# chsl/PLADE

Hardware: AMD Instinct MI355X
Metric: scan-pair registrations/sec, 1M-pt synthetic pairs (higher is better)
Workload: dtype f32

## Files before the change

plade_amd/csrc/ctx.h:

```cpp
#pragma once
#include "common.h"
#include "plade_hip.h"
#include "launch.h"
#include <ctime>
#include <sys/prctl.h>

namespace plade {

struct CloudDev {
    uint32_t n = 0;
    DBuf<float> soa;
    DBuf<float> aos;
    size_t pitch = 0;
    float bbmin[3] = {0, 0, 0}, bbmax[3] = {0, 0, 0};
    const float *x() const { return soa.p; }
    const float *y() const { return soa.p + pitch; }
    const float *z() const { return soa.p + 2 * pitch; }
    const float *nx() const { return soa.p + 3 * pitch; }
    const float *ny() const { return soa.p + 4 * pitch; }
    const float *nz() const { return soa.p + 5 * pitch; }
};

struct Stats {
    std::vector<std::string> names;
    std::vector<double> values;
    std::string joined;
    void clear() { names.clear(); values.clear(); }
    void add(const std::string &n, double v) {
        for (size_t i = 0; i < names.size(); ++i)
            if (names[i] == n) { values[i] += v; return; }
        names.push_back(n);
        values.push_back(v);
    }
    void merge(const Stats &o) { for (size_t i = 0; i < o.names.size(); ++i) add(o.names[i], o.values[i]); }
};

}

namespace plade {
inline void poll_sleep(int polls, bool crowd = false) {
    const long base_ns = crowd ? 100000L : 50000L;
    timespec ts{0, polls < 8 ? base_ns : 2 * base_ns};
    nanosleep(&ts, nullptr);
}
inline double thread_cpu_seconds() {
    timespec ts;
    clock_gettime(CLOCK_THREAD_CPUTIME_ID, &ts);
    return (double)ts.tv_sec + 1e-9 * (double)ts.tv_nsec;
}
inline void relax_timer_slack() {
    static thread_local bool done = false;
    if (!done) { (void)prctl(PR_SET_TIMERSLACK, 1000UL, 0, 0, 0); done = true; }
}
}

namespace plade {
struct ScanWork { DBuf<uint64_t> state; DBuf<uint32_t> ticket; uint32_t base = 0, gen = 0; };
struct VoxBatchWork { DBuf<uint32_t> keys, keys2, vals, vals2, heads, seg_group, offs; DBuf<float> sorted_xyz, obb_coef; };
}

namespace plade {
constexpr int COPY_OUT_RANGES = 8;
struct CopyOutArgs { const uint32_t *src[COPY_OUT_RANGES]; uint32_t off_words[COPY_OUT_RANGES], words[COPY_OUT_RANGES], n; };
void copy_out_launch(hipStream_t st, const CopyOutArgs &a, uint32_t *arena_words, uint32_t *counter, uint32_t *flag, uint32_t seq);
}

struct plade_cloud {
    plade::CloudDev dev;
    std::vector<float> host_copy;
};

namespace plade { struct RegistrationWork; struct RansacWork; struct NormalsWork; struct IcpWork; struct DistWork; struct OutlierWork; struct MergeWork; struct ComponentWork; }
namespace plade { void comm_all_gather_dev(plade_comm *c, const void *d_send, void *d_recv, size_t bytes, hipStream_t stream); }

struct plade_ctx {
    int device = 0;
    plade::RegistrationWork *reg_work = nullptr;
    plade::RansacWork *ransac_work = nullptr;
    plade::NormalsWork *normals_work = nullptr;
    plade::IcpWork *icp_work = nullptr;
    plade::DistWork *dist_work = nullptr;
    plade::OutlierWork *outlier_work = nullptr;
    plade::MergeWork *merge_work = nullptr;
    plade::ComponentWork *component_work = nullptr;
    plade_ctx *peers[PLADE_GROUP_MAX - 1] = {};
    hipEvent_t ev_group = nullptr;
    bool in_group = false;
    const char *stage_name = "";
    plade::Combiner *comb = nullptr;
    int comb_slot = -1;
    plade_ctx *aux = nullptr;
    hipStream_t stream = nullptr;
    plade::CloudDev up_tgt, up_src;
    struct Prefetch {
        hipStream_t stream = nullptr;
        plade::CloudDev cl[2 * PLADE_GROUP_MAX];
        const float *ptr[2 * PLADE_GROUP_MAX] = {};
        uint32_t n[2 * PLADE_GROUP_MAX] = {};
        int count = 0;
        bool valid = false;
        plade::HBuf<int> h;
        plade::DBuf<int> d;
    } pf;
    plade_params params;
    struct CandidateShard { uint32_t rank = 0, world = 1, min_candidates = 0; plade_exchange_fn exchange = nullptr; void *user = nullptr;
                            plade_comm *comm = nullptr;  } shard;
    uint64_t wait_epoch = 0;
    std::string last_error;
    std::map<std::string, std::vector<char>> dump;
    plade::Stats stats;
    struct EvRec { hipEvent_t a = nullptr, b = nullptr; std::string tag; double bytes = 0; int clk = -1; double clk_secs = -1.0; };
    std::vector<EvRec> evs;
    static constexpr int CLK_SLOTS = 1024, CLK_WAYS = 64;
    plade::DBuf<unsigned long long> clk_dev;
    int clk_used = 0;
    double clk_hz = 0;
    bool graph_clocks() const { return (params.dump & 6) == 6; }
    bool capturing = false;
    int cap_slot = 0;
    std::vector<std::string> cap_tags;
    std::vector<unsigned long long> clk_host, clk_init;
    void ensure_clk() {
        if (clk_dev.p) return;
        {
            clk_dev.ensure(2 * (size_t)CLK_SLOTS * CLK_WAYS);
            std::vector<unsigned long long> init(2 * (size_t)CLK_SLOTS * CLK_WAYS);
            for (size_t i = 0; i < init.size() / 2; ++i) { init[2 * i] = ~0ull; init[2 * i + 1] = 0ull; }
            (void)hipMemcpy(clk_dev.p, init.data(), init.size() * 8, hipMemcpyHostToDevice);
            int khz = 0;
            (void)hipDeviceGetAttribute(&khz, hipDeviceAttributeWallClockRate, device);
            clk_hz = khz > 0 ? khz * 1e3 : 1e8;
        }
    }
    unsigned long long *ev_clock() {
        if (graph_clocks()) {
            if (!capturing || cap_slot >= CLK_SLOTS) return nullptr;
            ensure_clk();
            return clk_dev.p + 2 * (size_t)CLK_WAYS * (cap_slot++);
        }
        if (!profiling() || evs.empty() || clk_used >= CLK_SLOTS) return nullptr;
        ensure_clk();
        evs.back().clk = clk_used;
        return clk_dev.p + 2 * (size_t)CLK_WAYS * (clk_used++);
    }
    void ev_graph_launched(const std::vector<std::string> &tags) {
        for (size_t j = 0; j < tags.size(); ++j) { EvRec r; r.tag = tags[j]; r.clk = (int)j; evs.push_back(r); }
    }
    void ev_graph_clocks(size_t ev0) {
        size_t used = 0;
        for (size_t e = ev0; e < evs.size(); ++e) if (!evs[e].a && evs[e].clk >= 0) used = std::max(used, (size_t)evs[e].clk + 1);
        if (!used) return;
        clk_host.resize(2 * used * CLK_WAYS);
        if (clk_init.size() < clk_host.size()) {
            clk_init.resize(clk_host.size());
            for (size_t i = 0; i < clk_init.size() / 2; ++i) { clk_init[2 * i] = ~0ull; clk_init[2 * i + 1] = 0ull; }
        }
        HIP_TRY(hipMemcpyAsync(clk_host.data(), clk_dev.p, clk_host.size() * 8, hipMemcpyDeviceToHost, stream));
        HIP_TRY(hipMemcpyAsync(clk_dev.p, clk_init.data(), clk_host.size() * 8, hipMemcpyHostToDevice, stream));
        HIP_TRY(hipStreamSynchronize(stream));
        for (size_t e = ev0; e < evs.size(); ++e) {
            EvRec &r = evs[e];
            if (r.a || r.clk < 0) continue;
            unsigned long long lo = ~0ull, hi = 0ull;
            for (int w = 0; w < CLK_WAYS; ++w) {
                lo = std::min(lo, clk_host[2 * ((size_t)r.clk * CLK_WAYS + w)]);
                hi = std::max(hi, clk_host[2 * ((size_t)r.clk * CLK_WAYS + w) + 1]);
            }
            r.clk_secs = hi > lo ? (double)(hi - lo) / clk_hz : -1.0;
            r.clk = -1;
        }
    }
    bool profiling() const { return (params.dump & 2) != 0; }
    void ev_begin(const char *tag, double bytes) {
        if (!profiling()) return;
        if (graph_clocks()) { if (capturing) cap_tags.push_back(tag); return; }
        EvRec r;
        r.tag = tag; r.bytes = bytes;
        (void)hipEventCreate(&r.a); (void)hipEventCreate(&r.b);
        (void)hipEventRecord(r.a, stream);
        evs.push_back(r);
    }
    void ev_end() {
        if (!profiling() || graph_clocks() || evs.empty()) return;
        (void)hipEventRecord(evs.back().b, stream);
    }
    void ev_collect() {
        if (evs.empty()) return;
        (void)hipStreamSynchronize(stream);
        std::vector<unsigned long long> clk(2 * (size_t)clk_used);
        if (clk_used) {
            std::vector<unsigned long long> raw(2 * (size_t)clk_used * CLK_WAYS);
            (void)hipMemcpy(raw.data(), clk_dev.p, raw.size() * 8, hipMemcpyDeviceToHost);
            for (int i = 0; i < clk_used; ++i) {
                unsigned long long lo = ~0ull, hi = 0ull;
                for (int w = 0; w < CLK_WAYS; ++w) {
                    lo = std::min(lo, raw[2 * ((size_t)i * CLK_WAYS + w)]);
                    hi = std::max(hi, raw[2 * ((size_t)i * CLK_WAYS + w) + 1]);
                }
                clk[2 * i] = lo; clk[2 * i + 1] = hi;
            }
            for (size_t i = 0; i < raw.size() / 2; ++i) { raw[2 * i] = ~0ull; raw[2 * i + 1] = 0ull; }
            (void)hipMemcpy(clk_dev.p, raw.data(), raw.size() * 8, hipMemcpyHostToDevice);
            clk_used = 0;
        }
        for (auto &r : evs) {
            float ms = 0.f;
            if (!r.a) {
                if (r.bytes >= 0 && r.clk_secs >= 0) {
                    stats.add("k_" + r.tag + "_seconds", r.clk_secs);
                    stats.add("k_" + r.tag + "_launches", 1.0);
                    stats.add("k_" + r.tag + "_bytes", r.bytes);
                    stats.add("k_" + r.tag + "_clock_seconds", r.clk_secs);
                    stats.add("k_" + r.tag + "_clock_launches", 1.0);
                    stats.add("k_" + r.tag + "_clock_bytes", r.bytes);
                } else stats.add("k_" + r.tag + "_idle_launches", 1.0);
                continue;
            }
            (void)hipEventElapsedTime(&ms, r.a, r.b);
            if (r.bytes >= 0) {
                stats.add("k_" + r.tag + "_seconds", ms * 1e-3);
                stats.add("k_" + r.tag + "_launches", 1.0);
                stats.add("k_" + r.tag + "_bytes", r.bytes);
                if (r.clk >= 0 && clk[2 * r.clk + 1] > clk[2 * r.clk]) {
                    stats.add("k_" + r.tag + "_clock_seconds", (double)(clk[2 * r.clk + 1] - clk[2 * r.clk]) / clk_hz);
                    stats.add("k_" + r.tag + "_clock_launches", 1.0);
                    stats.add("k_" + r.tag + "_clock_bytes", r.bytes);
                }
            } else stats.add("k_" + r.tag + "_idle_launches", 1.0);
            (void)hipEventDestroy(r.a); (void)hipEventDestroy(r.b);
        }
        evs.clear();
    }
    void sync(hipStream_t s = nullptr) {
        if (!s) s = stream;
        if (comb && s == stream) { comb->wait(this); return; }
        if (s == stream && !pending_reads.empty()) { sync_with_reads(); return; }
        if (params.host_wait == 0) { HIP_TRY(hipStreamSynchronize(s)); }
        else {
            plade::relax_timer_slack();
            const double c0 = plade::thread_cpu_seconds();
            struct Acc { plade::Stats &st; double c0; ~Acc() { st.add("cpu_sync_polls", plade::thread_cpu_seconds() - c0); } } acc{stats, c0};
            for (int polls = 0;; ++polls) {
                const hipError_t e = hipStreamQuery(s);
                if (e == hipSuccess) break;
                if (e != hipErrorNotReady) throw plade::Err{-2, std::string("hipStreamQuery: ") + hipGetErrorString(e)};
                plade::poll_sleep(polls, in_group);
            }
        }
        if (s == stream) { finish_reads(); write_arena_used = 0; ++wait_epoch; }
    }
    struct PendingRead { void *dst; const void *src; size_t off, bytes; std::vector<char> eager; };
    bool debug_reads = getenv("PLADE_DEBUG_READS") != nullptr;
    std::vector<PendingRead> pending_reads;
    plade::HBuf<char> read_arena;
    char *read_arena_dev = nullptr;
    plade::DBuf<uint32_t> read_counter;
    uint32_t read_seq = 0;
// ... 225 lines not shown
```

plade_amd/csrc/k_penetration.hip:

```cpp
#include "stages.h"
#include "prims.h"
#include "k_svd.h"
#include <algorithm>

namespace plade {

struct PenItem {
    uint32_t k, i1, j1;
    float plane1[4];
    float sx, sy, sz, dx, dy, dz, length;
};

struct PenTables {
    const float *cand;
    const float *s_coef;
    const float *s_center;
    const float *s_four;
    const float *t_coef;
    const float *t_center;
    const float *t_four;
    uint32_t K, ps, pt;
};

template <class Meet>
__device__ __forceinline__ void edge_hit(f3 lineVec, f3 linePoint, f3 a, f3 b, f3 *out, int &n, Meet meet) {
    const f3 tl = normalized_e(b - a);
    f3 ip;
    if (!meet(lineVec, linePoint, tl, a, ip)) return;
    if (dot_e(a - ip, b - ip) > 0) return;
    if (n < 4) out[n] = ip;
    ++n;
}
template <bool ROLLED, class Meet>
__device__ __forceinline__ int edge_hits(f3 lineVec, f3 linePoint, const f3 *c, f3 *out, Meet meet) {
    int n = 0;
    if (ROLLED) {
#pragma unroll 1
        for (int i = 1; i <= 4; ++i) edge_hit(lineVec, linePoint, c[(i - 1) % 4], c[i % 4], out, n, meet);
    } else {
        for (int i = 1; i <= 4; ++i) edge_hit(lineVec, linePoint, c[(i - 1) % 4], c[i % 4], out, n, meet);
    }
    return n;
}

struct PenTriple {
    uint32_t k, i1, j1;
    float plane1[4];
    f3 lineVec, linePoint;
    f3 c[8];
};

__device__ __forceinline__ bool pen_triple(const PenTables &tb, size_t idx, float len_th, float ang_th, PenTriple &t) {
    const uint32_t j1 = (uint32_t)(idx % tb.pt), i1 = (uint32_t)((idx / tb.pt) % tb.ps), k = (uint32_t)(idx / ((size_t)tb.pt * tb.ps));
    t.k = k; t.i1 = i1; t.j1 = j1;
    const float *c = tb.cand + 12 * (size_t)k;
    m3 R;
    for (int r = 0; r < 3; ++r) for (int q = 0; q < 3; ++q) R.m[r][q] = c[3 * r + q];
    const f3 T(c[9], c[10], c[11]);
    const float T12[12] = {c[0], c[1], c[2], c[9], c[3], c[4], c[5], c[10], c[6], c[7], c[8], c[11]};
    const float *sc = tb.s_coef + 4 * (size_t)i1;
    const f3 pn = mul_e(R, f3(sc[0], sc[1], sc[2]));
    t.plane1[0] = pn.x; t.plane1[1] = pn.y; t.plane1[2] = pn.z;
    t.plane1[3] = -(-sc[3] + dot_s(pn, T));
    const f3 c2m = mul_e(R, f3(tb.s_center[3 * i1], tb.s_center[3 * i1 + 1], tb.s_center[3 * i1 + 2])) + T;
    const float *tc = tb.t_coef + 4 * (size_t)j1;
    const f3 plane_A(tc[0], tc[1], tc[2]);
    const f3 tcen(tb.t_center[3 * j1], tb.t_center[3 * j1 + 1], tb.t_center[3 * j1 + 2]);
    const double c2p = (double)((fabsf(dot_e(plane_A, c2m) + tc[3]) + fabsf(dot_e(pn, tcen) + t.plane1[3])) / 2);
    if (c2p < (double)len_th && dot_e(pn, plane_A) > ang_th) return false;
    if (!plane_plane_line(t.plane1, tc, t.lineVec, t.linePoint)) return false;
    for (int q = 0; q < 4; ++q) {
        const float *f = tb.s_four + 12 * (size_t)i1 + 3 * q;
        t.c[q] = pcl_xform(T12, f3(f[0], f[1], f[2]));
        const float *g = tb.t_four + 12 * (size_t)j1 + 3 * q;
        t.c[4 + q] = f3(g[0], g[1], g[2]);
    }
    return true;
}

__device__ __forceinline__ void pen_emit(const PenTables &tb, const PenTriple &t, const f3 *ip1, const f3 *ip2, PenItem *__restrict__ items,
                                         uint32_t *__restrict__ pair_count) {
    const f3 direc = normalized_e(ip1[1] - ip1[0]);
    const f3 inter[4] = {ip1[0], ip1[1], ip2[0], ip2[1]};
    float len[4];
    int ord[4] = {0, 1, 2, 3};
    for (int q = 0; q < 4; ++q) len[q] = dot_e(inter[q] - inter[0], direc);
    for (int a = 1; a < 4; ++a) {
        int oi = ord[a];
        float lv = len[oi];
        int b = a - 1;
        while (b >= 0 && lv < len[ord[b]]) { ord[b + 1] = ord[b]; --b; }
        ord[b + 1] = oi;
    }
    if (0 == (ord[0] / 2 - ord[1] / 2)) return;
    const f3 sp = inter[ord[1]], ep = inter[ord[2]];
    const float length = norm_e(ep - sp);
    const uint32_t pair = t.i1 * tb.pt + t.j1;
    const uint32_t slot = pair * tb.K + atomicAdd(&pair_count[pair], 1u);
    PenItem it;
    it.k = t.k; it.i1 = t.i1; it.j1 = t.j1;
    for (int q = 0; q < 4; ++q) it.plane1[q] = t.plane1[q];
    it.sx = sp.x; it.sy = sp.y; it.sz = sp.z; it.dx = direc.x; it.dy = direc.y; it.dz = direc.z; it.length = length;
    items[slot] = it;
}

template <int TPB>
__device__ void k_pen_setup(const VB &vb, PenTables tb, float len_th, float ang_th, PenItem *__restrict__ items,
                            uint32_t *__restrict__ n_items, uint32_t *__restrict__ pair_count) {
    (void)n_items;
    const size_t idx = (size_t)vb.bx * blockDim.x + threadIdx.x;
    const size_t total = (size_t)tb.K * tb.ps * tb.pt;
    if (idx >= total) return;
    PenTriple t;
    if (!pen_triple(tb, idx, len_th, ang_th, t)) return;
    f3 ip1[4], ip2[4];
    auto meet = [&](f3 v1, f3 p1, f3 v2, f3 p2, f3 &out) -> bool { return lines_meet(v1, p1, v2, p2, out); };
    const int n1 = edge_hits<false>(t.lineVec, t.linePoint, t.c, ip1, meet);
    const int n2 = edge_hits<false>(t.lineVec, t.linePoint, t.c + 4, ip2, meet);
    if (n1 != 2 || n2 != 2) return;
    pen_emit(tb, t, ip1, ip2, items, pair_count);
}

constexpr int PS_TPB = 64;
__device__ void k_pen_setup_svd(const VB &vb, PenTables tb, float len_th, float ang_th, PenItem *__restrict__ items,
                                uint32_t *__restrict__ n_items, uint32_t *__restrict__ pair_count) {
    (void)n_items;
    __shared__ float pub[54 * PS_TPB];
    __shared__ uint16_t queue[8 * PS_TPB];
    const uint32_t lane = threadIdx.x;
    const size_t idx = (size_t)vb.bx * PS_TPB + lane;
    const size_t total = (size_t)tb.K * tb.ps * tb.pt;
    PenTriple t;
    const bool active = idx < total && pen_triple(tb, idx, len_th, ang_th, t);
    uint32_t need = 0;
    auto put = [&](int w, f3 v) { pub[(w + 0) * PS_TPB + lane] = v.x; pub[(w + 1) * PS_TPB + lane] = v.y; pub[(w + 2) * PS_TPB + lane] = v.z; };
    auto get = [&](int w, uint32_t l) { return f3(pub[(w + 0) * PS_TPB + l], pub[(w + 1) * PS_TPB + l], pub[(w + 2) * PS_TPB + l]); };
    if (active) {
        put(0, t.lineVec); put(3, t.linePoint);
#pragma unroll
        for (int e = 0; e < 8; ++e) {
            const int base = e & 4, i = (e & 3) + 1;
            const f3 a = t.c[base + (i - 1) % 4], b = t.c[base + i % 4];
            const f3 tl = normalized_e(b - a);
            if (!(fabsf(dot_e(t.lineVec, tl)) > 0.9999)) {
                need |= 1u << e;
                put(6 + 6 * e, tl); put(9 + 6 * e, a);
            }
        }
    }
    uint32_t n_items_wave = 0;
#pragma unroll
    for (int e = 0; e < 8; ++e) {
        const unsigned long long m = __ballot((need >> e) & 1u);
        if ((need >> e) & 1u) queue[n_items_wave + __popcll(m & ((1ull << lane) - 1ull))] = (uint16_t)(lane | (e << 6));
        n_items_wave += (uint32_t)__popcll(m);
    }
    __syncthreads();
    for (uint32_t first = 0; first < n_items_wave; first += PS_TPB) {
        const uint32_t it = first + lane;
        if (it < n_items_wave) {
            const uint32_t q = queue[it], sl = q & 63u, e = q >> 6;
            const f3 o = lines_meet_svd(get(0, sl), get(3, sl), get(6 + 6 * e, sl), get(9 + 6 * e, sl));
            pub[(6 + 6 * e) * PS_TPB + sl] = o.x; pub[(7 + 6 * e) * PS_TPB + sl] = o.y; pub[(8 + 6 * e) * PS_TPB + sl] = o.z;
        }
    }
    __syncthreads();
    if (!active) return;
    f3 ip1[4], ip2[4];
    int n1 = 0, n2 = 0;
#pragma unroll
    for (int e = 0; e < 8; ++e) {
        if (!((need >> e) & 1u)) continue;
        const int base = e & 4, i = (e & 3) + 1;
        const f3 a = t.c[base + (i - 1) % 4], b = t.c[base + i % 4];
        const f3 ip = get(6 + 6 * e, lane);
        if (dot_e(a - ip, b - ip) > 0) continue;
        if (e < 4) { if (n1 < 4) ip1[n1] = ip; ++n1; }
        else { if (n2 < 4) ip2[n2] = ip; ++n2; }
    }
    if (n1 != 2 || n2 != 2) return;
    pen_emit(tb, t, ip1, ip2, items, pair_count);
}

constexpr int PEN_MAXS = 1024;
constexpr int PEN_G = 4;
constexpr int PEN_TPB = 64 * PEN_G;

__device__ __forceinline__ void pen_uv(const PenFrame &f, f3 p, float &u, float &v) {
    const float dx = p.x - f.o[0], dy = p.y - f.o[1], dz = p.z - f.o[2];
    u = dx * f.eu[0] + dy * f.eu[1] + dz * f.eu[2];
    v = dx * f.ev[0] + dy * f.ev[1] + dz * f.ev[2];
}

__device__ void k_pen_cell_keys(const VB &vb, const float *__restrict__ xyz, uint32_t n, const uint32_t *__restrict__ off, uint32_t P,
                                const PenFrame *__restrict__ frames, float inv_cell, uint32_t *__restrict__ keys,
                                uint32_t *__restrict__ vals) {
    const uint32_t i = vb.bx * blockDim.x + threadIdx.x;
    if (i >= n) return;
    uint32_t lo = 0, hi = P;
    while (hi - lo > 1) { const uint32_t mid = (lo + hi) >> 1; if (off[mid] <= i) lo = mid; else hi = mid; }
    const PenFrame f = frames[lo];
    float u, v;
    pen_uv(f, f3(xyz[3 * (size_t)i], xyz[3 * (size_t)i + 1], xyz[3 * (size_t)i + 2]), u, v);
    const int cu = min(max((int)floorf(u * inv_cell) + 1, 0), f.nu - 1);
    const int cv = min(max((int)floorf(v * inv_cell) + 1, 0), f.nv - 1);
    keys[i] = f.base + (uint32_t)cv * (uint32_t)f.nu + (uint32_t)cu;
    vals[i] = i;
}

__device__ void k_pen_cell_fill(const VB &vb, const float *__restrict__ xyz, const uint32_t *__restrict__ skeys,
                                const uint32_t *__restrict__ svals, uint32_t n, uint32_t n_cells,
                                float4 *__restrict__ pts, uint32_t *__restrict__ cell_start) {
    const uint32_t i = vb.bx * blockDim.x + threadIdx.x;
    if (i < n) {
        const uint32_t p = svals[i];
        pts[i] = make_float4(xyz[3 * (size_t)p], xyz[3 * (size_t)p + 1], xyz[3 * (size_t)p + 2], 0.f);
    }
    if (i <= n_cells) {
        uint32_t lo = 0, hi = n;
        while (lo < hi) { const uint32_t mid = (lo + hi) >> 1; if (skeys[mid] < i) lo = mid + 1; else hi = mid; }
        cell_start[i] = lo;
    }
}

void build_pen_grid(plade_ctx *ctx, PlaneCloudsDev &pc, const PlaneGeomHost &geom, float cell) {
    const uint32_t P = geom.P, n = pc.off[P];
    std::vector<PenFrame> fr(P);
    uint32_t total = 0;
    for (uint32_t g = 0; g < P; ++g) {
        const float *c = geom.four.data() + 12 * (size_t)g;
        PenFrame &f = fr[g];
        double eu[3], ev[3], lu = 0, lv = 0;
        for (int k = 0; k < 3; ++k) { eu[k] = (double)c[3 + k] - c[k]; ev[k] = (double)c[9 + k] - c[k]; lu += eu[k] * eu[k]; lv += ev[k] * ev[k]; }
        lu = std::sqrt(lu); lv = std::sqrt(lv);
        for (int k = 0; k < 3; ++k) {
            f.o[k] = c[k];
            f.eu[k] = lu > 0 ? (float)(eu[k] / lu) : (k == 0);
            f.ev[k] = lv > 0 ? (float)(ev[k] / lv) : (k == 1);
        }
        f.nu = (int)std::min(4096.0, std::floor(lu / cell) + 3);
        f.nv = (int)std::min(4096.0, std::floor(lv / cell) + 3);
        f.base = total;
        total += (uint32_t)f.nu * (uint32_t)f.nv;
    }
    pc.n_cells = total;
    pc.grid_cell = cell;
    pc.frames.ensure(P);
    const bool staged = ctx->h2d(pc.frames.p, fr.data(), P * sizeof(PenFrame));
    pc.cell_pts.ensure((size_t)n + 1);
    pc.cell_start.ensure((size_t)total + 2);
    pc.ckeys.ensure((size_t)n + 1); pc.ckeys2.ensure((size_t)n + 1); pc.cvals.ensure((size_t)n + 1); pc.cvals2.ensure((size_t)n + 1);
    if (n)
        launch<k_pen_cell_keys, 256>(ctx, dim3(cdiv(n, 256)), 0, pc.xyz.p, n, pc.d_off.p, P, pc.frames.p,
                           1.f / cell, pc.ckeys.p, pc.cvals.p);
    int bits = 1;
    while ((1ull << bits) < total) ++bits;
    sort_pairs_u32(ctx, pc.ckeys.p, pc.ckeys2.p, pc.cvals.p, pc.cvals2.p, n, bits);
    launch<k_pen_cell_fill, 256>(ctx, dim3(cdiv(std::max(n, total + 1), 256)), 0, pc.xyz.p, pc.ckeys2.p,
                       pc.cvals2.p, n, total, pc.cell_pts.p, pc.cell_start.p);
    if (!staged) ctx->sync();
}

template <class Fn>
__device__ __forceinline__ void pen_visit(const PenFrame &f, const float4 *__restrict__ pts, const uint32_t *__restrict__ cell_start,
                                          f3 start, f3 direc, float L, float rr, float cell, int lane, Fn fn) {
    float su, sv, eu_, ev_;
    pen_uv(f, start, su, sv);
    pen_uv(f, f3(start.x + L * direc.x, start.y + L * direc.y, start.z + L * direc.z), eu_, ev_);
    const float inv = 1.f / cell;
    const bool major_u = fabsf(eu_ - su) >= fabsf(ev_ - sv);
    const float a0 = major_u ? su : sv, a1 = major_u ? eu_ : ev_, b0 = major_u ? sv : su, b1 = major_u ? ev_ : eu_;
    const int na = major_u ? f.nu : f.nv, nbm = major_u ? f.nv : f.nu;
    const float pad = rr * 1.4143f + 0.02f * cell;
    const float amin = fminf(a0, a1) - rr - 0.02f * cell, amax = fmaxf(a0, a1) + rr + 0.02f * cell;
    const int ca0 = max((int)floorf(amin * inv) + 1, 0), ca1 = min((int)floorf(amax * inv) + 1, na - 1);
    const float da = a1 - a0;
    const float slope = fabsf(da) > 1e-12f ? (b1 - b0) / da : 0.f;
    for (int base = ca0; base <= ca1; base += 64) {
        const int ca = base + lane;
        int cb0 = 0, ncell = 0;
        if (ca <= ca1) {
            float lo = fmaxf((float)(ca - 1) * cell, amin), hi = fminf((float)ca * cell, amax);
            if (hi < lo) { const float t = lo; lo = hi; hi = t; }
            const float bl = b0 + (lo - a0) * slope, bh = b0 + (hi - a0) * slope;
            cb0 = max((int)floorf((fminf(bl, bh) - pad) * inv) + 1, 0);
            const int cb1 = min((int)floorf((fmaxf(bl, bh) + pad) * inv) + 1, nbm - 1);
            ncell = max(cb1 - cb0 + 1, 0);
        }
        int most = ncell;
        for (int d = 32; d >= 1; d >>= 1) most = max(most, __shfl_xor(most, d, 64));
        constexpr int QN = 4;
        for (int q0 = 0; q0 < most; q0 += QN) {
            uint32_t pb[QN], len[QN], mine = 0;
#pragma unroll
            for (int q = 0; q < QN; ++q) {
                pb[q] = 0; len[q] = 0;
                if (q0 + q < ncell) {
                    const int cb = cb0 + q0 + q;
                    const uint32_t c = f.base + (major_u ? (uint32_t)cb * (uint32_t)f.nu + (uint32_t)ca
                                                         : (uint32_t)ca * (uint32_t)f.nu + (uint32_t)cb);
                    pb[q] = cell_start[c];
                    len[q] = cell_start[c + 1] - pb[q];
                }
                mine += len[q];
            }
            uint32_t incl = mine;
            for (int d = 1; d < 64; d <<= 1) { const uint32_t o = __shfl_up(incl, d, 64); if (lane >= d) incl += o; }
            const uint32_t total = __shfl(incl, 63, 64), excl = incl - mine;
            for (uint32_t t0 = 0; t0 < total; t0 += 64) {
                const uint32_t t = t0 + (uint32_t)lane;
                int lo = 0, hi = 63;
                for (int it = 0; it < 6; ++it) {
                    const int mid = (lo + hi) >> 1;
                    const bool right = __shfl(incl, mid, 64) <= t;
                    lo = right ? mid + 1 : lo;
                    hi = right ? hi : mid;
                }
                uint32_t r = t - __shfl(excl, lo, 64), at = 0;
                bool found = false;
#pragma unroll
                for (int q = 0; q < QN; ++q) {
                    const uint32_t o_pb = __shfl(pb[q], lo, 64), o_len = __shfl(len[q], lo, 64);
                    if (!found && r < o_len) { at = o_pb + r; found = true; }
                    if (!found) r -= o_len;
                }
                if (t < total && found) {
                    const float4 p4 = pts[at];
                    fn(f3(p4.x, p4.y, p4.z));
                }
            }
        }
    }
}

struct PenSide {
    const PenFrame *frames;
    const float4 *pts;
    const uint32_t *cell_start;
};

__device__ void k_pen_walk(const VB &vb, const PenItem *__restrict__ items, const uint32_t *__restrict__ pair_count,
                                                      const uint32_t *__restrict__ pair_order, PenTables tb,
                                                      const float *__restrict__ step_dist, PenSide S, PenSide T_, float cell,
                                                      float search_radius, int min_points, float min_distance,
                                                      uint32_t *__restrict__ cand_flags, uint32_t *__restrict__ overflow) {
    __shared__ uint32_t s_cnt_all[PEN_G][PEN_MAXS];
    __shared__ float s_dist[PEN_MAXS + 1];
    const uint32_t pair = pair_order[vb.bx];
    const uint32_t cnt = pair_count[pair];
    if (vb.by * PEN_G >= cnt) return;
    for (int i = threadIdx.x; i <= PEN_MAXS; i += blockDim.x) s_dist[i] = step_dist[i];
    __syncthreads();
    const int wave = __builtin_amdgcn_readfirstlane((int)(threadIdx.x >> 6)), lane = threadIdx.x & 63;
    const uint32_t slot = vb.by * PEN_G + wave;
    if (slot >= cnt) return;
    uint32_t *s_cnt = s_cnt_all[wave];
    const PenItem it = items[(size_t)pair * tb.K + slot];
    if (__atomic_load_n(&cand_flags[it.k], __ATOMIC_RELAXED)) return;
    int nsteps;
    {
        int lo = 0, hi = PEN_MAXS;
        while (lo < hi) { const int mid = (lo + hi) >> 1; if (s_dist[mid] < it.length) lo = mid + 1; else hi = mid; }
        if (lo == PEN_MAXS && s_dist[PEN_MAXS] < it.length && lane == 0) atomicExch(overflow, 1u);
        nsteps = lo;
    }
    if (nsteps == 0) return;
    const f3 start(it.sx, it.sy, it.sz), direc(it.dx, it.dy, it.dz);
    const float half_r2 = (float)((double)(search_radius / 2) * (double)(search_radius / 2));
    const float full_r2 = (float)((double)search_radius * (double)search_radius);
    const float *c = tb.cand + 12 * (size_t)it.k;
    const float T12[12] = {c[0], c[1], c[2], c[9], c[3], c[4], c[5], c[10], c[6], c[7], c[8], c[11]};
    const uint32_t i1 = pair / tb.pt, j1 = pair % tb.pt;
    const float *tc = tb.t_coef + 4 * (size_t)j1;
    const float inv_r = 1.f / search_radius;
    const float L = s_dist[nsteps - 1];
    const f3 ds(start.x - c[9], start.y - c[10], start.z - c[11]);
    const f3 start_s(c[0] * ds.x + c[3] * ds.y + c[6] * ds.z, c[1] * ds.x + c[4] * ds.y + c[7] * ds.z,
                     c[2] * ds.x + c[5] * ds.y + c[8] * ds.z);
    const f3 direc_s(c[0] * direc.x + c[3] * direc.y + c[6] * direc.z, c[1] * direc.x + c[4] * direc.y + c[7] * direc.z,
                     c[2] * direc.x + c[5] * direc.y + c[8] * direc.z);
    const PenFrame fs = S.frames[i1], ft = T_.frames[j1];

    for (int pass = 0; pass < 2; ++pass) {
        for (int i = lane; i < nsteps; i += 64) s_cnt[i] = 0u;
        __syncwarp();
        auto gate = [&](f3 raw) {
            const f3 p = pass == 0 ? raw : pcl_xform(T12, raw);
            const f3 d = p - start;
            const float t = d.x * direc.x + d.y * direc.y + d.z * direc.z;
            const int kc = (int)floorf(t * inv_r);
            for (int kk = max(kc - 2, 0); kk <= min(kc + 3, nsteps - 1); ++kk) {
                const float dist = s_dist[kk];
                const f3 spt(start.x + dist * direc.x, start.y + dist * direc.y, start.z + dist * direc.z);
                if (flann_d2(spt, p) < half_r2) atomicAdd(&s_cnt[kk], 1u);
            }
        };
        if (pass == 0) pen_visit(ft, T_.pts, T_.cell_start, start, direc, L, search_radius * 0.5f, cell, lane, gate);
        else pen_visit(fs, S.pts, S.cell_start, start_s, direc_s, L, search_radius * 0.5f, cell, lane, gate);
        __syncwarp();
        if (__atomic_load_n(&cand_flags[it.k], __ATOMIC_RELAXED)) return;
        const float pl0 = pass == 0 ? tc[0] : it.plane1[0], pl1 = pass == 0 ? tc[1] : it.plane1[1],
                    pl2 = pass == 0 ? tc[2] : it.plane1[2], pl3 = pass == 0 ? tc[3] : it.plane1[3];
        int pos = 0, neg = 0;
        auto classify = [&](f3 raw) {
            const f3 p = pass == 0 ? pcl_xform(T12, raw) : raw;
            const f3 d = p - start;
            const float t = d.x * direc.x + d.y * direc.y + d.z * direc.z;
            const int kc = (int)floorf(t * inv_r);
            bool hit = false;
            for (int kk = max(kc - 2, 0); kk <= min(kc + 3, nsteps - 1) && !hit; ++kk) {
                if (s_cnt[kk] < 2u) continue;
                const float dist = s_dist[kk];
                const f3 spt(start.x + dist * direc.x, start.y + dist * direc.y, start.z + dist * direc.z);
                if (flann_d2(spt, p) < full_r2) hit = true;
            }
            if (hit) {
                const float td = pl0 * p.x + pl1 * p.y + pl2 * p.z + pl3;
                if (fabsf(td) > min_distance) { if (td >= 0) ++pos; else ++neg; }
            }
        };
        if (pass == 0) pen_visit(fs, S.pts, S.cell_start, start_s, direc_s, L, search_radius, cell, lane, classify);
        else pen_visit(ft, T_.pts, T_.cell_start, start, direc, L, search_radius, cell, lane, classify);
        for (int dlt = 32; dlt >= 1; dlt >>= 1) { pos += __shfl_xor(pos, dlt, 64); neg += __shfl_xor(neg, dlt, 64); }
        __syncwarp();
        if (pass == 0) {
            if (pos < min_points || neg < min_points) return;
        } else {
            if (pos < min_points && neg < min_points) return;
        }
        if ((double)max(pos, neg) / (double)min(pos, neg + 1) > 5) return;
    }
    if (lane == 0) atomicOr(&cand_flags[it.k], 1u);
}

void penetration_filter(plade_ctx *ctx, const float *cand_rt_host, uint32_t K, const PlaneGeomHost &src,
                        const PlaneGeomHost &tgt, PlaneCloudsDev &src_pts, PlaneCloudsDev &tgt_pts,
                        float length_threshold, float angle_threshold, std::vector<int32_t> &flags_out, const float *cand_rt_dev,
                        const PenGather *gather) {
    flags_out.assign(K, 0);
    if (!K || !src.P || !tgt.P) {
        if (gather && K) {
            uint32_t *d_ids = reinterpret_cast<uint32_t *>(ctx->scratch[4].ensure(4 * (size_t)K + 64));
            ctx->h2d(d_ids, gather->ids, 4 * (size_t)K);
            gather->launch(d_ids);
        }
        if (cand_rt_dev) ctx->sync();
        return;
    }
    const uint32_t n_pairs = src.P * tgt.P;
    const size_t n_cand = cand_rt_dev ? 0 : 12 * (size_t)K;
    const size_t n_tab = n_cand + (4 + 3 + 12) * ((size_t)src.P + tgt.P);
    const size_t n_ids = gather ? K : 0;
    const size_t n_ctr = (size_t)K + 2 + n_pairs;
    const size_t nf = n_tab + (PEN_MAXS + 1) + n_pairs + n_ids + n_ctr;
    std::vector<float> h(nf, 0.f);
    float *p = h.data();
    if (n_cand) memcpy(p, cand_rt_host, 48 * (size_t)K);
    float *o_cand = p; p += n_cand;
    float *o_sc = p; memcpy(p, src.coef.data(), 16 * (size_t)src.P); p += 4 * (size_t)src.P;
    float *o_scen = p; memcpy(p, src.center.data(), 12 * (size_t)src.P); p += 3 * (size_t)src.P;
    float *o_sf = p; memcpy(p, src.four.data(), 48 * (size_t)src.P); p += 12 * (size_t)src.P;
    float *o_tc = p; memcpy(p, tgt.coef.data(), 16 * (size_t)tgt.P); p += 4 * (size_t)tgt.P;
    float *o_tcen = p; memcpy(p, tgt.center.data(), 12 * (size_t)tgt.P); p += 3 * (size_t)tgt.P;
    float *o_tf = p; memcpy(p, tgt.four.data(), 48 * (size_t)tgt.P); p += 12 * (size_t)tgt.P;
    float *d = reinterpret_cast<float *>(ctx->scratch[4].ensure(nf * 4 + 64));
    PenTables tb;
    tb.cand = cand_rt_dev ? cand_rt_dev : d + (o_cand - h.data()); tb.s_coef = d + (o_sc - h.data()); tb.s_center = d + (o_scen - h.data());
    tb.s_four = d + (o_sf - h.data()); tb.t_coef = d + (o_tc - h.data()); tb.t_center = d + (o_tcen - h.data());
    tb.t_four = d + (o_tf - h.data());
    tb.K = K; tb.ps = src.P; tb.pt = tgt.P;
    const size_t total = (size_t)K * src.P * tgt.P;
    PLADE_REQUIRE(total < (1ull << 31), PLADE_ELIMIT, "penetration: too many (candidate, plane, plane) triples");
    PenItem *d_items = reinterpret_cast<PenItem *>(ctx->scratch[5].ensure(total * sizeof(PenItem) + 64));
    const float search_radius = (float)(double)length_threshold;
    const float min_distance = (float)((double)length_threshold / 2);
    uint32_t *d_ctr = reinterpret_cast<uint32_t *>(d + n_tab + PEN_MAXS + 1 + n_pairs + n_ids);
    uint32_t *d_n = d_ctr, *d_over = d_ctr + 1, *d_flags = d_ctr + 2, *d_pair = d_ctr + 2 + K;
    std::vector<uint32_t> order(n_pairs);
    {
        std::vector<uint32_t> w(n_pairs);
        for (uint32_t i = 0; i < src.P; ++i)
            for (uint32_t j = 0; j < tgt.P; ++j)
                w[i * tgt.P + j] = (src_pts.off[i + 1] - src_pts.off[i]) + (tgt_pts.off[j + 1] - tgt_pts.off[j]);
        for (uint32_t i = 0; i < n_pairs; ++i) order[i] = i;
        std::stable_sort(order.begin(), order.end(), [&](uint32_t a, uint32_t b) { return w[a] > w[b]; });
    }
    float *h_steps = h.data() + n_tab;
    {
        float dist = 0;
        for (int i = 0; i <= PEN_MAXS; ++i) { h_steps[i] = dist; dist += search_radius; }
    }
    memcpy(h.data() + n_tab + PEN_MAXS + 1, order.data(), 4 * (size_t)n_pairs);
    if (n_ids) memcpy(h.data() + n_tab + PEN_MAXS + 1 + n_pairs, gather->ids, 4 * n_ids);
    ctx->h2d(d, h.data(), nf * 4);
    if (gather) gather->launch(reinterpret_cast<const uint32_t *>(d + n_tab + PEN_MAXS + 1 + n_pairs));
    const float *d_steps = d + n_tab;
    const uint32_t *d_order = reinterpret_cast<const uint32_t *>(d + n_tab + PEN_MAXS + 1);
    if (ctx->params.closest_point_mode == 1)
        launch<k_pen_setup_svd, PS_TPB>(ctx, dim3(cdiv(total, PS_TPB)), 0, tb, length_threshold,
                           angle_threshold, d_items, d_n, d_pair);
    else
        launch<k_pen_setup<256>, 256>(ctx, dim3(cdiv(total, 256)), 0, tb, length_threshold,
                           angle_threshold, d_items, d_n, d_pair);
    const float cell = pen_grid_cell(length_threshold);
    if (src_pts.grid_cell != cell) build_pen_grid(ctx, src_pts, src, cell);
    if (tgt_pts.grid_cell != cell) build_pen_grid(ctx, tgt_pts, tgt, cell);
    const PenSide sS{src_pts.frames.p, src_pts.cell_pts.p, src_pts.cell_start.p}, sT{tgt_pts.frames.p, tgt_pts.cell_pts.p, tgt_pts.cell_start.p};
    ctx->ev_begin("pen_walk", 0.0);
    launch<k_pen_walk, PEN_TPB, 6>(ctx, dim3(n_pairs, cdiv(K, PEN_G)), 0, d_items, d_pair, d_order, tb, d_steps,
                       sS, sT, cell, search_radius, 10, min_distance, d_flags, d_over);
    ctx->ev_end();
    std::vector<uint32_t> out(n_ctr);
    ctx->d2h(out.data(), d_ctr, n_ctr * 4);
    ctx->sync();
    HIP_TRY(hipGetLastError());
    double items = 0;
    for (uint32_t pr = 0; pr < n_pairs; ++pr) items += out[(size_t)K + 2 + pr];
    ctx->stats.add("pen_items", items);
    PLADE_REQUIRE(out[1] == 0, PLADE_ELIMIT, "penetration: intersection segment longer than 1024 search steps");
    for (uint32_t k = 0; k < K; ++k) flags_out[k] = out[k + 2] ? 1 : 0;
}

}
```

Measured before the change: 905.0.

## Compact penetration walk grid, split setup solves into phases, add early gating

The penetration walk kernel now, by default, launches a small persistent grid of workgroups. Each workgroup builds a prefix-sum table over per-pair item counts and binary-searches it to map virtual blocks onto occupied (pair, slot) work, instead of launching a dense n_pairs x K/G grid where most blocks exit at once. The SVD setup kernel handles the two quads in two phases and stops early when no lane survives the first quad, which halves its shared memory footprint. The walk also skips the plane-side test when no step cell holds at least two points, and optional diagnostic counters are gated by an environment variable. The risks are a per-block table build and search overhead, less parallelism from capping the grid at 256 workgroups, and a possible behaviour change from the new gating early-return.

```diff
diff --git a/plade_amd/csrc/ctx.h b/plade_amd/csrc/ctx.h
--- a/plade_amd/csrc/ctx.h
+++ b/plade_amd/csrc/ctx.h
@@ -69,6 +69,19 @@
     plade::CloudDev dev;
     std::vector<float> host_copy;
 };
+
+namespace plade {
+struct PenOpts {
+    uint32_t table_max = 1024;
+    bool count = false;
+    static PenOpts from_env() {
+        PenOpts o;
+        if (const char *w = getenv("PLADE_PEN_TABLE_MAX")) { const int v = atoi(w); o.table_max = (uint32_t)(v < 0 ? 0 : v > 1024 ? 1024 : v); }
+        o.count = getenv("PLADE_PEN_COUNT") != nullptr;
+        return o;
+    }
+};
+}
 
 namespace plade { struct RegistrationWork; struct RansacWork; struct NormalsWork; struct IcpWork; struct DistWork; struct OutlierWork; struct MergeWork; struct ComponentWork; }
 namespace plade { void comm_all_gather_dev(plade_comm *c, const void *d_send, void *d_recv, size_t bytes, hipStream_t stream); }
@@ -103,6 +116,7 @@
         plade::DBuf<int> d;
     } pf;
     plade_params params;
+    const plade::PenOpts pen_opts = plade::PenOpts::from_env();
     struct CandidateShard { uint32_t rank = 0, world = 1, min_candidates = 0; plade_exchange_fn exchange = nullptr; void *user = nullptr;
                             plade_comm *comm = nullptr;  } shard;
     uint64_t wait_epoch = 0;
diff --git a/plade_amd/csrc/k_penetration.hip b/plade_amd/csrc/k_penetration.hip
--- a/plade_amd/csrc/k_penetration.hip
+++ b/plade_amd/csrc/k_penetration.hip
@@ -122,63 +122,83 @@
 }
 
 constexpr int PS_TPB = 64;
+enum { PD_SURVIVORS, PD_N1_IS_2, PD_N2_IS_2, PD_SOLVES, PD_WALKED, PD_SKIP0, PD_SKIP1, PD_MAX_STEPS, PD_WORDS };
+__device__ __forceinline__ void pen_diag_add(uint32_t *diag, int what, bool pred, uint32_t lane) {
+    const uint32_t n = (uint32_t)__popcll(__ballot(pred));
+    if (lane == 0 && n) atomicAdd(&diag[what], n);
+}
+
+template <bool COUNT>
 __device__ void k_pen_setup_svd(const VB &vb, PenTables tb, float len_th, float ang_th, PenItem *__restrict__ items,
-                                uint32_t *__restrict__ n_items, uint32_t *__restrict__ pair_count) {
-    (void)n_items;
-    __shared__ float pub[54 * PS_TPB];
-    __shared__ uint16_t queue[8 * PS_TPB];
+                                uint32_t *__restrict__ diag, uint32_t *__restrict__ pair_count) {
+    __shared__ float pub[30 * PS_TPB];
+    __shared__ uint16_t queue[4 * PS_TPB];
     const uint32_t lane = threadIdx.x;
     const size_t idx = (size_t)vb.bx * PS_TPB + lane;
     const size_t total = (size_t)tb.K * tb.ps * tb.pt;
     PenTriple t;
     const bool active = idx < total && pen_triple(tb, idx, len_th, ang_th, t);
-    uint32_t need = 0;
     auto put = [&](int w, f3 v) { pub[(w + 0) * PS_TPB + lane] = v.x; pub[(w + 1) * PS_TPB + lane] = v.y; pub[(w + 2) * PS_TPB + lane] = v.z; };
     auto get = [&](int w, uint32_t l) { return f3(pub[(w + 0) * PS_TPB + l], pub[(w + 1) * PS_TPB + l], pub[(w + 2) * PS_TPB + l]); };
-    if (active) {
-        put(0, t.lineVec); put(3, t.linePoint);
-#pragma unroll
-        for (int e = 0; e < 8; ++e) {
-            const int base = e & 4, i = (e & 3) + 1;
-            const f3 a = t.c[base + (i - 1) % 4], b = t.c[base + i % 4];
-            const f3 tl = normalized_e(b - a);
-            if (!(fabsf(dot_e(t.lineVec, tl)) > 0.9999)) {
-                need |= 1u << e;
-                put(6 + 6 * e, tl); put(9 + 6 * e, a);
-            }
-        }
-    }
-    uint32_t n_items_wave = 0;
-#pragma unroll
-    for (int e = 0; e < 8; ++e) {
-        const unsigned long long m = __ballot((need >> e) & 1u);
-        if ((need >> e) & 1u) queue[n_items_wave + __popcll(m & ((1ull << lane) - 1ull))] = (uint16_t)(lane | (e << 6));
-        n_items_wave += (uint32_t)__popcll(m);
-    }
-    __syncthreads();
-    for (uint32_t first = 0; first < n_items_wave; first += PS_TPB) {
-        const uint32_t it = first + lane;
-        if (it < n_items_wave) {
-            const uint32_t q = queue[it], sl = q & 63u, e = q >> 6;
-            const f3 o = lines_meet_svd(get(0, sl), get(3, sl), get(6 + 6 * e, sl), get(9 + 6 * e, sl));
-            pub[(6 + 6 * e) * PS_TPB + sl] = o.x; pub[(7 + 6 * e) * PS_TPB + sl] = o.y; pub[(8 + 6 * e) * PS_TPB + sl] = o.z;
-        }
-    }
-    __syncthreads();
-    if (!active) return;
-    f3 ip1[4], ip2[4];
-    int n1 = 0, n2 = 0;
-#pragma unroll
-    for (int e = 0; e < 8; ++e) {
-        if (!((need >> e) & 1u)) continue;
-        const int base = e & 4, i = (e & 3) + 1;
-        const f3 a = t.c[base + (i - 1) % 4], b = t.c[base + i % 4];
-        const f3 ip = get(6 + 6 * e, lane);
-        if (dot_e(a - ip, b - ip) > 0) continue;
-        if (e < 4) { if (n1 < 4) ip1[n1] = ip; ++n1; }
-        else { if (n2 < 4) ip2[n2] = ip; ++n2; }
-    }
-    if (n1 != 2 || n2 != 2) return;
+    if (active) { put(0, t.lineVec); put(3, t.linePoint); }
+    if (COUNT) pen_diag_add(diag, PD_SURVIVORS, active, lane);
+    bool live = active;
+    f3 ip1[2], ip2[2];
+#pragma unroll 1
+    for (int ph = 0; ph < 2; ++ph) {
+        if (__ballot(live) == 0ull) return;
+        const f3 *c4 = t.c;
+        uint32_t need = 0;
+        if (live) {
+#pragma unroll
+            for (int q = 0; q < 4; ++q) {
+                const f3 a = c4[q], b = c4[(q + 1) % 4];
+                const f3 tl = normalized_e(b - a);
+                if (!(fabsf(dot_e(t.lineVec, tl)) > 0.9999)) {
+                    need |= 1u << q;
+                    put(6 + 6 * q, tl); put(9 + 6 * q, a);
+                }
+            }
+        }
+        uint32_t n_items_wave = 0;
+#pragma unroll
+        for (int q = 0; q < 4; ++q) {
+            const unsigned long long m = __ballot((need >> q) & 1u);
+            if ((need >> q) & 1u) queue[n_items_wave + __popcll(m & ((1ull << lane) - 1ull))] = (uint16_t)(lane | (q << 6));
+            n_items_wave += (uint32_t)__popcll(m);
+        }
+        if (COUNT && lane == 0) atomicAdd(&diag[PD_SOLVES], n_items_wave);
+        __syncthreads();
+        for (uint32_t first = 0; first < n_items_wave; first += PS_TPB) {
+            const uint32_t it = first + lane;
+            if (it < n_items_wave) {
+                const uint32_t qe = queue[it], sl = qe & 63u, q = qe >> 6;
+                const f3 o = lines_meet_svd(get(0, sl), get(3, sl), get(6 + 6 * q, sl), get(9 + 6 * q, sl));
+                pub[(6 + 6 * q) * PS_TPB + sl] = o.x; pub[(7 + 6 * q) * PS_TPB + sl] = o.y; pub[(8 + 6 * q) * PS_TPB + sl] = o.z;
+            }
+        }
+        __syncthreads();
+        int n = 0;
+        if (live) {
+#pragma unroll
+            for (int q = 0; q < 4; ++q) {
+                if (!((need >> q) & 1u)) continue;
+                const f3 a = c4[q], b = c4[(q + 1) % 4];
+                const f3 ip = get(6 + 6 * q, lane);
+                if (dot_e(a - ip, b - ip) > 0) continue;
+                if (n == 0) ip2[0] = ip; else if (n == 1) ip2[1] = ip;
+                ++n;
+            }
+        }
+        if (COUNT) pen_diag_add(diag, ph ? PD_N2_IS_2 : PD_N1_IS_2, live && n == 2, lane);
+        live = live && n == 2;
+        if (ph == 0) {
+            ip1[0] = ip2[0]; ip1[1] = ip2[1];
+#pragma unroll
+            for (int q = 0; q < 4; ++q) t.c[q] = t.c[4 + q];
+        }
+    }
+    if (!live) return;
     pen_emit(tb, t, ip1, ip2, items, pair_count);
 }
 
@@ -339,22 +359,60 @@
     const uint32_t *cell_start;
 };
 
+constexpr int PEN_TABLE = 1024;
+constexpr uint32_t PEN_WGS = 256;
+
+__device__ __forceinline__ uint32_t pen_grid_build(const uint32_t *__restrict__ pair_count, const uint32_t *__restrict__ pair_order,
+                                                   uint32_t n_pairs, uint32_t *s_start , uint32_t *s_wsum ) {
+    static_assert(PEN_TABLE == 4 * PEN_TPB, "four table entries per lane");
+    const uint32_t t = threadIdx.x, lane = t & 63u, w = t >> 6;
+    uint32_t v[4], sum = 0;
+#pragma unroll
+    for (int q = 0; q < 4; ++q) {
+        const uint32_t b = 4 * t + q;
+        v[q] = b < n_pairs ? (pair_count[pair_order[b]] + PEN_G - 1) / PEN_G : 0u;
+        sum += v[q];
+    }
+    uint32_t incl = sum;
+#pragma unroll
+    for (int d = 1; d < 64; d <<= 1) { const uint32_t o = __shfl_up(incl, d, 64); if (lane >= (uint32_t)d) incl += o; }
+    if (lane == 63) s_wsum[w] = incl;
+    __syncthreads();
+    uint32_t run = incl - sum;
+    for (uint32_t q = 0; q < w; ++q) run += s_wsum[q];
+#pragma unroll
+    for (int q = 0; q < 4; ++q) { s_start[4 * t + q] = run; run += v[q]; }
+    if (t == PEN_TPB - 1) s_start[PEN_TABLE] = run;
+    __syncthreads();
+    return s_start[PEN_TABLE];
+}
+__device__ __forceinline__ uint32_t pen_grid_find(const uint32_t *s_start, uint32_t n_pairs, uint32_t vt) {
+    uint32_t lo = 0, hi = n_pairs;
+    while (hi - lo > 1) { const uint32_t mid = (lo + hi) >> 1; if (s_start[mid] <= vt) lo = mid; else hi = mid; }
+    return lo;
+}
+
+template <bool COUNT>
 __device__ void k_pen_walk(const VB &vb, const PenItem *__restrict__ items, const uint32_t *__restrict__ pair_count,
                                                       const uint32_t *__restrict__ pair_order, PenTables tb,
                                                       const float *__restrict__ step_dist, PenSide S, PenSide T_, float cell,
                                                       float search_radius, int min_points, float min_distance,
-                                                      uint32_t *__restrict__ cand_flags, uint32_t *__restrict__ overflow) {
+                                                      uint32_t *__restrict__ cand_flags, uint32_t *__restrict__ overflow,
+                                                      uint32_t n_pairs, uint32_t compact_grid, uint32_t *__restrict__ diag) {
     __shared__ uint32_t s_cnt_all[PEN_G][PEN_MAXS];
     __shared__ float s_dist[PEN_MAXS + 1];
-    const uint32_t pair = pair_order[vb.bx];
-    const uint32_t cnt = pair_count[pair];
-    if (vb.by * PEN_G >= cnt) return;
+    __shared__ uint32_t s_start[PEN_TABLE + 1];
+    __shared__ uint32_t s_wsum[PEN_G];
+    const bool compact = compact_grid != 0u;
+    if (!compact && vb.by * PEN_G >= pair_count[pair_order[vb.bx]]) return;
     for (int i = threadIdx.x; i <= PEN_MAXS; i += blockDim.x) s_dist[i] = step_dist[i];
-    __syncthreads();
+    uint32_t n_virtual = 0;
+    if (compact) n_virtual = __builtin_amdgcn_readfirstlane(pen_grid_build(pair_count, pair_order, n_pairs, s_start, s_wsum));
+    else __syncthreads();
     const int wave = __builtin_amdgcn_readfirstlane((int)(threadIdx.x >> 6)), lane = threadIdx.x & 63;
-    const uint32_t slot = vb.by * PEN_G + wave;
-    if (slot >= cnt) return;
     uint32_t *s_cnt = s_cnt_all[wave];
+
+    auto walk = [&](const uint32_t pair, const uint32_t slot) __attribute__((always_inline)) {
     const PenItem it = items[(size_t)pair * tb.K + slot];
     if (__atomic_load_n(&cand_flags[it.k], __ATOMIC_RELAXED)) return;
     int nsteps;
@@ -399,6 +457,16 @@
         else pen_visit(fs, S.pts, S.cell_start, start_s, direc_s, L, search_radius * 0.5f, cell, lane, gate);
         __syncwarp();
         if (__atomic_load_n(&cand_flags[it.k], __ATOMIC_RELAXED)) return;
+        bool gated = false;
+        for (int base = 0; base < nsteps; base += 64) {
+            const int i = base + lane;
+            gated = gated || __ballot(i < nsteps && s_cnt[i] >= 2u) != 0ull;
+        }
+        if (COUNT && pass == 0 && lane == 0) { atomicAdd(&diag[PD_WALKED], 1u); atomicMax(&diag[PD_MAX_STEPS], (uint32_t)nsteps); }
+        if (!gated) {
+            if (COUNT && lane == 0) atomicAdd(&diag[pass == 0 ? PD_SKIP0 : PD_SKIP1], 1u);
+            return;
+        }
         const float pl0 = pass == 0 ? tc[0] : it.plane1[0], pl1 = pass == 0 ? tc[1] : it.plane1[1],
                     pl2 = pass == 0 ? tc[2] : it.plane1[2], pl3 = pass == 0 ? tc[3] : it.plane1[3];
         int pos = 0, neg = 0;
@@ -431,6 +499,20 @@
         if ((double)max(pos, neg) / (double)min(pos, neg + 1) > 5) return;
     }
     if (lane == 0) atomicOr(&cand_flags[it.k], 1u);
+    };
+
+    for (uint32_t vt = vb.bx;; vt += vb.gx) {
+        uint32_t pair, slot;
+        if (compact) {
+            if (vt >= n_virtual) break;
+            const uint32_t b = __builtin_amdgcn_readfirstlane(pen_grid_find(s_start, n_pairs, vt));
+            pair = pair_order[b]; slot = (vt - (uint32_t)__builtin_amdgcn_readfirstlane(s_start[b])) * PEN_G + wave;
+        } else {
+            pair = pair_order[vb.bx]; slot = vb.by * PEN_G + wave;
+        }
+        if (slot < pair_count[pair]) walk(pair, slot);
+        if (!compact) break;
+    }
 }
 
 void penetration_filter(plade_ctx *ctx, const float *cand_rt_host, uint32_t K, const PlaneGeomHost &src,
@@ -451,7 +533,8 @@
     const size_t n_cand = cand_rt_dev ? 0 : 12 * (size_t)K;
     const size_t n_tab = n_cand + (4 + 3 + 12) * ((size_t)src.P + tgt.P);
     const size_t n_ids = gather ? K : 0;
-    const size_t n_ctr = (size_t)K + 2 + n_pairs;
+    const PenOpts &po = ctx->pen_opts;
+    const size_t n_ctr = (size_t)K + 2 + n_pairs + PD_WORDS;
     const size_t nf = n_tab + (PEN_MAXS + 1) + n_pairs + n_ids + n_ctr;
     std::vector<float> h(nf, 0.f);
     float *p = h.data();
@@ -475,7 +558,7 @@
     const float search_radius = (float)(double)length_threshold;
     const float min_distance = (float)((double)length_threshold / 2);
     uint32_t *d_ctr = reinterpret_cast<uint32_t *>(d + n_tab + PEN_MAXS + 1 + n_pairs + n_ids);
-    uint32_t *d_n = d_ctr, *d_over = d_ctr + 1, *d_flags = d_ctr + 2, *d_pair = d_ctr + 2 + K;
+    uint32_t *d_over = d_ctr + 1, *d_flags = d_ctr + 2, *d_pair = d_ctr + 2 + K, *d_diag = d_pair + n_pairs;
     std::vector<uint32_t> order(n_pairs);
     {
         std::vector<uint32_t> w(n_pairs);
@@ -496,19 +579,27 @@
     if (gather) gather->launch(reinterpret_cast<const uint32_t *>(d + n_tab + PEN_MAXS + 1 + n_pairs));
     const float *d_steps = d + n_tab;
     const uint32_t *d_order = reinterpret_cast<const uint32_t *>(d + n_tab + PEN_MAXS + 1);
-    if (ctx->params.closest_point_mode == 1)
-        launch<k_pen_setup_svd, PS_TPB>(ctx, dim3(cdiv(total, PS_TPB)), 0, tb, length_threshold,
-                           angle_threshold, d_items, d_n, d_pair);
-    else
+    if (ctx->params.closest_point_mode == 1) {
+        const dim3 g(cdiv(total, PS_TPB));
+        if (po.count) launch<k_pen_setup_svd<true>, PS_TPB>(ctx, g, 0, tb, length_threshold, angle_threshold, d_items, d_diag, d_pair);
+        else launch<k_pen_setup_svd<false>, PS_TPB>(ctx, g, 0, tb, length_threshold, angle_threshold, d_items, d_diag, d_pair);
+    } else
         launch<k_pen_setup<256>, 256>(ctx, dim3(cdiv(total, 256)), 0, tb, length_threshold,
-                           angle_threshold, d_items, d_n, d_pair);
+                           angle_threshold, d_items, d_diag, d_pair);
     const float cell = pen_grid_cell(length_threshold);
     if (src_pts.grid_cell != cell) build_pen_grid(ctx, src_pts, src, cell);
     if (tgt_pts.grid_cell != cell) build_pen_grid(ctx, tgt_pts, tgt, cell);
     const PenSide sS{src_pts.frames.p, src_pts.cell_pts.p, src_pts.cell_start.p}, sT{tgt_pts.frames.p, tgt_pts.cell_pts.p, tgt_pts.cell_start.p};
+    const uint32_t dense_y = cdiv(K, PEN_G);
+    const bool compact = n_pairs <= po.table_max;
+    const dim3 grid = compact ? dim3((uint32_t)std::min<uint64_t>(PEN_WGS, (uint64_t)n_pairs * dense_y)) : dim3(n_pairs, dense_y);
     ctx->ev_begin("pen_walk", 0.0);
-    launch<k_pen_walk, PEN_TPB, 6>(ctx, dim3(n_pairs, cdiv(K, PEN_G)), 0, d_items, d_pair, d_order, tb, d_steps,
-                       sS, sT, cell, search_radius, 10, min_distance, d_flags, d_over);
+    if (po.count)
+        launch<k_pen_walk<true>, PEN_TPB, 6>(ctx, grid, 0, d_items, d_pair, d_order, tb, d_steps, sS, sT, cell, search_radius, 10,
+                           min_distance, d_flags, d_over, n_pairs, compact ? 1u : 0u, d_diag);
+    else
+        launch<k_pen_walk<false>, PEN_TPB, 6>(ctx, grid, 0, d_items, d_pair, d_order, tb, d_steps, sS, sT, cell, search_radius, 10,
+                           min_distance, d_flags, d_over, n_pairs, compact ? 1u : 0u, d_diag);
     ctx->ev_end();
     std::vector<uint32_t> out(n_ctr);
     ctx->d2h(out.data(), d_ctr, n_ctr * 4);
@@ -517,6 +608,32 @@
     double items = 0;
     for (uint32_t pr = 0; pr < n_pairs; ++pr) items += out[(size_t)K + 2 + pr];
     ctx->stats.add("pen_items", items);
+    if (po.count) {
+        const uint32_t *dg = out.data() + (size_t)K + 2 + n_pairs;
+        double empty_pairs = 0, partial = 0, wgs_items = 0;
+        for (uint32_t pr = 0; pr < n_pairs; ++pr) {
+            const uint32_t c = out[(size_t)K + 2 + pr];
+            empty_pairs += c == 0;
+            partial += c % PEN_G != 0;
+            wgs_items += cdiv(c, (uint32_t)PEN_G);
+        }
+        ctx->stats.add("pen_diag_triples", (double)total);
+        ctx->stats.add("pen_diag_plane_pairs", (double)n_pairs);
+        ctx->stats.add("pen_diag_gate_survivors", dg[PD_SURVIVORS]);
+        ctx->stats.add("pen_diag_n1_is_2", dg[PD_N1_IS_2]);
+        ctx->stats.add("pen_diag_n2_is_2", dg[PD_N2_IS_2]);
+        ctx->stats.add("pen_diag_solves", dg[PD_SOLVES]);
+        ctx->stats.add("pen_diag_items_walked", dg[PD_WALKED]);
+        ctx->stats.add("pen_diag_skipped_pass0", dg[PD_SKIP0]);
+        ctx->stats.add("pen_diag_skipped_pass1", dg[PD_SKIP1]);
+        ctx->stats.add("pen_diag_max_steps", dg[PD_MAX_STEPS]);
+        ctx->stats.add("pen_diag_pairs_without_items", empty_pairs);
+        ctx->stats.add("pen_diag_pairs_with_partial_workgroup", partial);
+        ctx->stats.add("pen_diag_walk_workgroups_with_items", wgs_items);
+        ctx->stats.add("pen_diag_walk_workgroups_dense", (double)n_pairs * dense_y);
+        ctx->stats.add("pen_diag_walk_workgroups_launched", (double)grid.x * grid.y);
+        ctx->stats.add("pen_diag_compact_grid", compact ? 1.0 : 0.0);
+    }
     PLADE_REQUIRE(out[1] == 0, PLADE_ELIMIT, "penetration: intersection segment longer than 1024 search steps");
     for (uint32_t k = 0; k < K; ++k) flags_out[k] = out[k + 2] ? 1 : 0;
 }
```

Measured after the change: 878.3. 0.971x the previous value.
